# ruc-aimc-lab/GeoFormer

Measured on NVIDIA B200. Metric: pairs_per_sec_640x480, higher is better.
Workload: dtype tf32 / fp16 tensor-core operands with fp32 accumulation (fp32 residual stream, fp16 intermediates), split-fp16 similarity, f16 backbone activations

## Files before the change

geoformer_b200/_lib.py:

```python
from __future__ import annotations

import ctypes
import os
from ctypes import c_char_p, c_float, c_int, c_int64, c_void_p

HERE = os.path.dirname(os.path.abspath(__file__))
LIB_PATH = os.path.join(HERE, "libgeoformer_sm100.so")

P, I, L, F = c_void_p, c_int, c_int64, c_float

SIGNATURES = {
    "gf_abi_version": (I, []),
    "gf_last_error": (c_char_p, []),
    "gf_init": (I, [I]),
    "gf_launch_count": (L, []),
    "gf_linear_tf32": (I, [P, P, P, P, L, I, I, I, I, I, P, P, I, P, P, P, P, P]),
    "gf_linear_ref": (I, [P, P, P, P, L, I, I, I, I, I, P, P, I, P, P, P, P, P]),
    "gf_conv3x3_f16": (I, [P, P, P, P, P, I, I, I, I, I, I, I, P]),
    "gf_conv_f16": (I, [P, P, P, P, P, I, I, I, I, I, I, I, I, I, P]),
    "gf_stem_conv7x7_f16": (I, [P, P, P, P, I, I, I, P]),
    "gf_upsample_add_f16": (I, [P, P, P, I, I, I, I, I, I, P]),
    "gf_conv_ref": (I, [P, P, P, P, P, I, I, I, I, I, I, I, I, P]),
    "gf_upsample_add_ref": (I, [P, P, P, I, I, I, I, I, I, P]),
    "gf_add_posenc": (I, [P, P, P, I, L, I, P]),
    "gf_linattn_partial_floats": (L, [I, I, I, I]),
    "gf_linear_mixed": (I, [P, P, P, P, I, I, L, I, I, I, I, I, P, P, I, P, P, P, P, P]),
    "gf_fine_layer": (I, [P, P, P, P, P, P, P, P, L, P]),
    "gf_linattn_reduce_f16": (I, [P, I, P, I, I, I, I, I, P, P, P, P]),
    "gf_linattn_apply_f16": (I, [P, I, P, P, P, I, I, I, I, I, P]),
    "gf_linattn_window_f16": (I, [P, I, P, I, P, I, P, L, I, I, I, P]),
    "gf_linattn_reduce": (I, [P, I, P, I, I, I, I, I, P, P, P, P]),
    "gf_linattn_apply": (I, [P, I, P, P, P, I, I, I, I, I, P]),
    "gf_linattn_window": (I, [P, I, P, I, P, I, P, L, I, I, I, P]),
    "gf_pack_split_f16": (I, [P, P, L, I, F, I, P]),
    "gf_similarity_f16x3": (I, [P, P, P, I, I, I, I, F, P]),
    "gf_similarity_ref": (I, [P, P, P, I, I, I, I, F, F, P]),
    "gf_dual_softmax_workspace_floats": (L, [I, I, I]),
    "gf_dual_softmax_stats": (I, [P, I, I, I, P, P, P, P, P, P]),
    "gf_dual_softmax_conf": (I, [P, I, I, I, P, P, P, P, P, P, P]),
    "gf_conf_row_col_max": (I, [P, I, I, I, P, P, P]),
    "gf_mnn_select": (I, [P, I, I, I, F, I, I, I, I, I, P, P, P, P, P]),
    "gf_coarse_match_fused_workspace_bytes": (L, [I, I, I]),
    "gf_coarse_match_fused": (I, [P, P, I, I, I, I, F, F, I, I, I, I, I, P, P, P, P]),
    "gf_coarse_match_fused_pass": (I, [P, P, I, I, I, I, F, P, I, P]),
    "gf_compact_coarse": (I, [P, P, I, I, I, I, F, P, P, P, P, P, P, P, P, L, P]),
    "gf_geo_window_table": (I, [P, P, I, I, I, I, I, I, I, I, P, P]),
    "gf_geo_self_attention": (I, [P, I, P, I, P, I, P, I, I, I, I, P, P, I, P]),
    "gf_gather_anchor_kv": (I, [P, I, P, I, I, I, I, I, P, P, I, I, P, P, P]),
    "gf_gather_anchor_kv_f16": (I, [P, I, P, I, P, I, I, I, I, I, P, P, I, I, P, P, P, P]),
    "gf_geo_self_attention_tc": (I, [P, I, P, P, P, I, I, I, I, I, P, P]),
    "gf_gather_anchor_kv_h16": (I, [P, I, P, I, I, I, I, I, P, P, I, I, P, P, P]),
    "gf_masked_softmax_rows": (I, [P, I, I, I, I, P, P]),
    "gf_gemm_tf32_batched": (I, [P, L, L, P, L, L, P, L, L, I, I, I, I, F, P]),
    "gf_geo_cross_attention": (I, [P, I, P, I, P, I, P, I, I, I, I, I, P, I, P]),
    "gf_geo_cross_attention_f16": (I, [P, I, P, I, P, I, P, I, I, I, I, I, P, I, P]),
    "gf_select_rows": (I, [P, P, P, I, L, I, P]),
    "gf_fine_gather": (I, [P, I, I, I, P, P, L, I, I, I, P, P]),
# ... 60 lines not shown
```

geoformer_b200/csrc/conv_tc.cu:

```cuda
#include "common.cuh"
#include "ptx.cuh"

#include <atomic>
#include <cstdlib>
#include <cuda_fp16.h>

namespace gf {
extern std::atomic<int64_t> g_launches;

struct ConvParams {
  const float* bias;
  const __half* residual;
  int batch, h, w, cout_p;
  int kbc;
  int last_k;
  int tail;
  int taps, stride, pad;
  int tiles_x, tiles_y;
  int act;
};

template <int BN, int MT = 1> struct ConvCfg {
  static constexpr int kStageA = MT * 128 * 128;
  static constexpr int kStageB = (BN / 2) * 128;
// ... 253 lines not shown
                                         float ry, float rx) {
  const int64_t idx = (int64_t)blockIdx.x * blockDim.x + threadIdx.x;
  const int64_t total = (int64_t)b * h * w * c8;
  if (idx >= total) return;
  const int ch = (int)(idx % c8);
  int64_t r = idx / c8;
  const int x = (int)(r % w); r /= w;
  const int y = (int)(r % h);
  const int n = (int)(r / h);
  const float fy = ry * y, fx = rx * x;
  const int y0 = (int)fy, x0 = (int)fx;
  const int y1 = min(y0 + 1, hs - 1), x1 = min(x0 + 1, ws - 1);
  const float ly = fy - y0, lx = fx - x0;
  const float w00 = (1.f - ly) * (1.f - lx), w01 = (1.f - ly) * lx, w10 = ly * (1.f - lx), w11 = ly * lx;
  const uint4* s = src + (int64_t)n * hs * ws * c8;
  const uint4 a = __ldg(s + ((int64_t)y0 * ws + x0) * c8 + ch), bq = __ldg(s + ((int64_t)y0 * ws + x1) * c8 + ch);
  const uint4 cq = __ldg(s + ((int64_t)y1 * ws + x0) * c8 + ch), d = __ldg(s + ((int64_t)y1 * ws + x1) * c8 + ch);
  const uint4 l = __ldg(lateral + idx);
  const uint32_t aw[4] = {a.x, a.y, a.z, a.w}, bw[4] = {bq.x, bq.y, bq.z, bq.w}, cw[4] = {cq.x, cq.y, cq.z, cq.w},
                 dw[4] = {d.x, d.y, d.z, d.w}, lw[4] = {l.x, l.y, l.z, l.w};
  uint32_t o[4];
#pragma unroll
  for (int q = 0; q < 4; ++q) {
    const __half2 a2 = *reinterpret_cast<const __half2*>(&aw[q]), b2 = *reinterpret_cast<const __half2*>(&bw[q]);
    const __half2 c2 = *reinterpret_cast<const __half2*>(&cw[q]), d2 = *reinterpret_cast<const __half2*>(&dw[q]);
    const __half2 l2 = *reinterpret_cast<const __half2*>(&lw[q]);
    const float lo = __low2float(l2) + w00 * __low2float(a2) + w01 * __low2float(b2) + w10 * __low2float(c2) + w11 * __low2float(d2);
    const float hi = __high2float(l2) + w00 * __high2float(a2) + w01 * __high2float(b2) + w10 * __high2float(c2) + w11 * __high2float(d2);
    o[q] = pack_f16(lo, hi);
  }
  out[idx] = make_uint4(o[0], o[1], o[2], o[3]);
}

__global__ void __launch_bounds__(256)
stem_conv7x7_kernel(const float* __restrict__ img, const float* __restrict__ wperm, const float* __restrict__ bias,
                    __half* __restrict__ out, int h, int w, int ho, int wo) {
  __shared__ float patch[21][72];
  __shared__ __align__(16) float ws[49 * 128];
  const int b = blockIdx.z;
  const int oy0 = blockIdx.y * 8, ox0 = blockIdx.x * 32;
  const int tid = threadIdx.x;
  for (int e = tid; e < 49 * 128; e += 256) ws[e] = wperm[e];
  const int iy0 = oy0 * 2 - 3, ix0 = ox0 * 2 - 3;
  const float* im = img + (int64_t)b * h * w;
  for (int e = tid; e < 21 * 69; e += 256) {
    const int r = e / 69, c = e - r * 69;
    const int y = iy0 + r, x = ix0 + c;
    patch[r][c] = (y >= 0 && y < h && x >= 0 && x < w) ? im[(int64_t)y * w + x] : 0.f;
  }
  __syncthreads();
  const int cg = tid & 7, pg = tid >> 3;
  const int prow = pg >> 2, pcol = (pg & 3) * 8;
  float acc[8][16];
#pragma unroll
  for (int i = 0; i < 8; ++i)
#pragma unroll
    for (int j = 0; j < 16; ++j) acc[i][j] = 0.f;
#pragma unroll 1
  for (int ky = 0; ky < 7; ++ky) {
    float in[21];
#pragma unroll
    for (int i = 0; i < 21; ++i) in[i] = patch[prow * 2 + ky][pcol * 2 + i];
#pragma unroll
    for (int kx = 0; kx < 7; ++kx) {
      const float4* wp = reinterpret_cast<const float4*>(ws + (ky * 7 + kx) * 128) + cg;
#pragma unroll
      for (int j = 0; j < 4; ++j) {
        const float4 w4 = wp[j * 8];
#pragma unroll
        for (int i = 0; i < 8; ++i) {
          const float x = in[2 * i + kx];
          acc[i][4 * j] = fmaf(x, w4.x, acc[i][4 * j]); acc[i][4 * j + 1] = fmaf(x, w4.y, acc[i][4 * j + 1]);
          acc[i][4 * j + 2] = fmaf(x, w4.z, acc[i][4 * j + 2]); acc[i][4 * j + 3] = fmaf(x, w4.w, acc[i][4 * j + 3]);
        }
      }
    }
  }
  const int oy = oy0 + prow;
  if (oy < ho) {
#pragma unroll
    for (int j = 0; j < 4; ++j) {
      const float4 b4 = __ldg(reinterpret_cast<const float4*>(bias + j * 32 + cg * 4));
#pragma unroll
      for (int i = 0; i < 8; ++i) {
        const int ox = ox0 + pcol + i;
        if (ox < wo) {
          uint2 o;
          o.x = pack_f16(fmaxf(acc[i][4 * j] + b4.x, 0.f), fmaxf(acc[i][4 * j + 1] + b4.y, 0.f));
          o.y = pack_f16(fmaxf(acc[i][4 * j + 2] + b4.z, 0.f), fmaxf(acc[i][4 * j + 3] + b4.w, 0.f));
          *reinterpret_cast<uint2*>(out + (((int64_t)b * ho + oy) * wo + ox) * 128 + j * 32 + cg * 4) = o;
        }
      }
    }
  }
}

typedef CUresult (*EncodeTiledFn)(CUtensorMap*, CUtensorMapDataType, cuuint32_t, void*, const cuuint64_t*,
                                  const cuuint64_t*, const cuuint32_t*, const cuuint32_t*, CUtensorMapInterleave,
                                  CUtensorMapSwizzle, CUtensorMapL2promotion, CUtensorMapFloatOOBfill);
EncodeTiledFn encode_fn();

static int make_nhwc_tmap(CUtensorMap* m, const void* base, int c, int w, int h, int b, int box_w, int box_h, int stride = 1,
                          int box_c = 64) {
  EncodeTiledFn enc = encode_fn();
  if (!enc) return gf_set_error(GF_ERR_DRIVER, "gf_init() was not called");
  cuuint64_t dims[4] = {(cuuint64_t)c, (cuuint64_t)w, (cuuint64_t)h, (cuuint64_t)b};
  cuuint64_t strides[3] = {(cuuint64_t)c * 2, (cuuint64_t)c * 2 * w, (cuuint64_t)c * 2 * w * h};
  cuuint32_t box[4] = {(cuuint32_t)box_c, (cuuint32_t)(box_w * stride), (cuuint32_t)(box_h * stride), 1};
  cuuint32_t estr[4] = {1, (cuuint32_t)stride, (cuuint32_t)stride, 1};
  CUresult r = enc(m, CU_TENSOR_MAP_DATA_TYPE_FLOAT16, 4, const_cast<void*>(base), dims, strides, box, estr,
                   CU_TENSOR_MAP_INTERLEAVE_NONE, box_c == 64 ? CU_TENSOR_MAP_SWIZZLE_128B : CU_TENSOR_MAP_SWIZZLE_32B,
                   CU_TENSOR_MAP_L2_PROMOTION_L2_256B, CU_TENSOR_MAP_FLOAT_OOB_FILL_NONE);
  if (r != CUDA_SUCCESS) return gf_set_error(GF_ERR_DRIVER, "cuTensorMapEncodeTiled(nhwc) failed");
  return GF_OK;
}

static int make_wtail_tmap(CUtensorMap* m, const void* base, int64_t k, int64_t rows, int box_rows) {
  EncodeTiledFn enc = encode_fn();
  if (!enc) return gf_set_error(GF_ERR_DRIVER, "gf_init() was not called");
  cuuint64_t dims[3] = {(cuuint64_t)k, (cuuint64_t)rows, 1};
  cuuint64_t strides[2] = {(cuuint64_t)k * 2, (cuuint64_t)k * 2 * (cuuint64_t)rows};
  cuuint32_t box[3] = {16, (cuuint32_t)box_rows, 1};
  cuuint32_t estr[3] = {1, 1, 1};
// ... 55 lines not shown
    if ((rc = make_wtail_tmap(&twt, wt, taps * (int64_t)cin_k, cout_p, BN / 2))) return rc;
  }
  p.tiles_x = gf_cdiv(wo, 16); p.tiles_y = gf_cdiv(ho, 8); p.act = act;
  if (BN == 128 && ho >= 32 && getenv("GF_CONV_MT1") == nullptr) {
    p.tiles_y = gf_cdiv(ho, 16);
    return launch_conv<128, 2>(tx, tw, ty, txt, twt, p, (cudaStream_t)stream);
  }
  if (BN == 128) return launch_conv<128>(tx, tw, ty, txt, twt, p, (cudaStream_t)stream);
  if (BN == 208) return launch_conv<208>(tx, tw, ty, txt, twt, p, (cudaStream_t)stream);
  return launch_conv<256>(tx, tw, ty, txt, twt, p, (cudaStream_t)stream);
}

extern "C" int gf_conv3x3_f16(const void* x, const void* wt, const float* bias, const void* residual, void* y,
                               int batch, int h, int w, int cin_p, int cout_p, int cin_k, int act, gf_stream_t stream) {
  return gf_conv_f16(x, wt, bias, residual, y, batch, h, w, cin_p, cout_p, cin_k, 3, 1, act, stream);
}

extern "C" int gf_upsample_add_f16(const void* lateral, const void* src, void* out, int batch, int h, int w, int hs,
                                    int ws, int c, gf_stream_t stream) {
  if (batch <= 0 || h <= 1 || w <= 1 || hs <= 0 || ws <= 0 || (c % 8)) return gf_set_error(GF_ERR_ARG, "gf_upsample_add_f16: bad shape");
  const int64_t total = (int64_t)batch * h * w * (c / 8);
  const float ry = (float)(hs - 1) / (float)(h - 1), rx = (float)(ws - 1) / (float)(w - 1);
  upsample_add_f16_kernel<<<gf_cdiv(total, 256), 256, 0, (cudaStream_t)stream>>>(
      (const uint4*)lateral, (const uint4*)src, (uint4*)out, batch, h, w, hs, ws, c / 8, ry, rx);
  g_launches++;
  GF_CHECK_LAUNCH();
  return GF_OK;
}

extern "C" int gf_stem_conv7x7_f16(const float* img, const float* wperm, const float* bias, void* out, int batch, int h,
                                    int w, gf_stream_t stream) {
  if (batch <= 0 || h <= 0 || w <= 0) return gf_set_error(GF_ERR_ARG, "gf_stem_conv7x7_f16: bad shape");
  const int ho = (h + 6 - 7) / 2 + 1, wo = (w + 6 - 7) / 2 + 1;
  stem_conv7x7_kernel<<<dim3(gf_cdiv(wo, 32), gf_cdiv(ho, 8), batch), 256, 0, (cudaStream_t)stream>>>(
      img, wperm, bias, (__half*)out, h, w, ho, wo);
  g_launches++;
  GF_CHECK_LAUNCH();
  return GF_OK;
}
```

geoformer_b200/csrc/linattn.cu:

```cuda
#include "common.cuh"

#include <cuda_fp16.h>

#include <atomic>

namespace gf {
extern std::atomic<int64_t> g_launches;

template <typename T> __device__ __forceinline__ float4 ld4(const T* p);
template <> __device__ __forceinline__ float4 ld4<float>(const float* p) { return *reinterpret_cast<const float4*>(p); }
template <> __device__ __forceinline__ float4 ld4<__half>(const __half* p) {
  const uint2 u = *reinterpret_cast<const uint2*>(p);
  const float2 a = __half22float2(*reinterpret_cast<const __half2*>(&u.x));
  const float2 b = __half22float2(*reinterpret_cast<const __half2*>(&u.y));
  return make_float4(a.x, a.y, b.x, b.y);
}
__device__ __forceinline__ void st1(float* p, float v) { *p = v; }
__device__ __forceinline__ void st1(__half* p, float v) { *p = __float2half_rn(v); }

constexpr int kChunk = 256;
constexpr int kChunkMma = 128;

template <int D, typename T>
__global__ void linattn_partial_kernel(const T* __restrict__ K, int ldk, const T* __restrict__ V, int ldv,
// ... 407 lines not shown
  __syncthreads();
  float ksr[D];
#pragma unroll
  for (int d = 0; d < D; ++d) ksr[d] = ksum[h * D + d];
  __half* os = reinterpret_cast<__half*>(vs);
#pragma unroll 5
  for (int r = 0; r < TOK; ++r) {
    const float4* qr = reinterpret_cast<const float4*>(qs + r * c + h * D);
    float num = 0.f, den = 0.f;
#pragma unroll
    for (int q = 0; q < D / 4; ++q) {
      const float4 q4 = qr[q];
      num = fmaf(q4.x, kvcol[4 * q], num); den = fmaf(q4.x, ksr[4 * q], den);
      num = fmaf(q4.y, kvcol[4 * q + 1], num); den = fmaf(q4.y, ksr[4 * q + 1], den);
      num = fmaf(q4.z, kvcol[4 * q + 2], num); den = fmaf(q4.z, ksr[4 * q + 2], den);
      num = fmaf(q4.w, kvcol[4 * q + 3], num); den = fmaf(q4.w, ksr[4 * q + 3], den);
    }
    os[r * c + t] = __float2half_rn(num * (1.f / (den + 1e-6f)) * ftok);
  }
  __syncthreads();
  uint4* dst = reinterpret_cast<uint4*>(out + w * (TOK * c));
  const uint4* src = reinterpret_cast<const uint4*>(os);
  for (int i = t; i < TOK * c / 8; i += 128) dst[i] = src[i];
}

__global__ void add_posenc_kernel(const float4* __restrict__ x, const float4* __restrict__ pe, float4* __restrict__ out,
                                  int64_t per_sample4, int64_t total4) {
  const int64_t i = (int64_t)blockIdx.x * blockDim.x + threadIdx.x;
  if (i >= total4) return;
  const float4 a = x[i], b = pe[i % per_sample4];
  out[i] = make_float4(a.x + b.x, a.y + b.y, a.z + b.z, a.w + b.w);
}

__global__ void select_rows_kernel(float4* __restrict__ dst, const float4* __restrict__ src, const int* __restrict__ flag,
                                   int64_t per_sample4, int64_t total4) {
  const int64_t i = (int64_t)blockIdx.x * blockDim.x + threadIdx.x;
  if (i >= total4) return;
  if (flag[i / per_sample4] == 0) dst[i] = src[i];
}

__global__ void gather_rows_kernel(const float* __restrict__ feat, int64_t l, int c, const int64_t* __restrict__ b_ids,
                                   const int64_t* __restrict__ tok, int64_t m, float* __restrict__ out) {
  const int64_t i = (int64_t)blockIdx.x * blockDim.x + threadIdx.x;
  const int c4 = c >> 2;
  if (i >= m * c4) return;
  const int64_t r = i / c4;
  const int q = (int)(i - r * c4);
  const float4* src = reinterpret_cast<const float4*>(feat + (b_ids[r] * l + tok[r]) * c);
  reinterpret_cast<float4*>(out)[i] = src[q];
}

}

using namespace gf;
#define STREAM ((cudaStream_t)stream)

extern "C" int64_t gf_linattn_partial_floats(int n, int s, int heads, int dim) {
  return (int64_t)n * heads * gf_cdiv(s, kChunkMma) * (dim * dim + dim);
}

template <typename T>
static int linattn_reduce_impl(const T* K, int ldk, const T* V, int ldv, int n, int s, int heads, int dim,
                               float* partial, float* KV, float* Ksum, gf_stream_t stream) {
  if (n <= 0 || s <= 0 || heads <= 0 || heads > 32 || dim != 32 || (ldk % 4) || (ldv % 4))
    return gf_set_error(GF_ERR_ARG, "gf_linattn_reduce: dim must be 32, heads <= 32, 16-byte aligned rows");
  const int nchunks = gf_cdiv(s, kChunk);
// ... 65 lines not shown
  linattn_window16_kernel<16, 25><<<(unsigned)n_windows, 128, smem, STREAM>>>((const __half*)Q, ldq, (const __half*)K, ldk,
                                                                            (const __half*)V, ldv, (__half*)out);
  g_launches++;
  GF_CHECK_LAUNCH();
  return GF_OK;
}

extern "C" int gf_linattn_window(const float* Q, int ldq, const float* K, int ldk, const float* V, int ldv, float* out,
                                 int64_t n_windows, int tokens, int heads, int dim, gf_stream_t stream) {
  const int c = heads * dim;
  if (n_windows < 0 || tokens <= 0 || tokens > 64 || dim != 16 || c > 1024 || (c % 32))
    return gf_set_error(GF_ERR_ARG, "gf_linattn_window: dim must be 16");
  if (n_windows == 0) return GF_OK;
  const size_t smem = (size_t)(3 * tokens * c + c) * sizeof(float);
  GF_SMEM_OPTIN((linattn_window_kernel<16, 0>), 96 * 1024);
  GF_SMEM_OPTIN((linattn_window_kernel<16, 25>), 96 * 1024);
  if (smem > 96 * 1024) return gf_set_error(GF_ERR_ARG, "gf_linattn_window: shared memory");
  if (tokens == 25) linattn_window_kernel<16, 25><<<(unsigned)n_windows, c, smem, STREAM>>>(Q, ldq, K, ldk, V, ldv, out, tokens, heads);
  else              linattn_window_kernel<16, 0><<<(unsigned)n_windows, c, smem, STREAM>>>(Q, ldq, K, ldk, V, ldv, out, tokens, heads);
  g_launches++;
  GF_CHECK_LAUNCH();
  return GF_OK;
}

extern "C" int gf_add_posenc(const float* x, const float* pe, float* out, int n, int64_t l, int c, gf_stream_t stream) {
  if (n <= 0 || l <= 0 || c <= 0 || (c % 4)) return gf_set_error(GF_ERR_ARG, "gf_add_posenc: bad shape");
  const int64_t per = l * c / 4, total = per * n;
  add_posenc_kernel<<<gf_cdiv(total, 256), 256, 0, STREAM>>>((const float4*)x, (const float4*)pe, (float4*)out, per, total);
  g_launches++;
  GF_CHECK_LAUNCH();
  return GF_OK;
}

extern "C" int gf_select_rows(float* dst, const float* src, const int* flag, int n, int64_t l, int c, gf_stream_t stream) {
  if (n <= 0 || l <= 0 || c <= 0 || (c % 4)) return gf_set_error(GF_ERR_ARG, "gf_select_rows: bad shape");
  const int64_t per = l * c / 4, total = per * n;
  select_rows_kernel<<<gf_cdiv(total, 256), 256, 0, STREAM>>>((float4*)dst, (const float4*)src, flag, per, total);
  g_launches++;
  GF_CHECK_LAUNCH();
  return GF_OK;
}

extern "C" int gf_gather_rows(const float* feat, int64_t l, int c, const int64_t* b_ids, const int64_t* tok_ids,
                              int64_t m, float* out, gf_stream_t stream) {
  if (m < 0 || c <= 0 || (c % 4)) return gf_set_error(GF_ERR_ARG, "gf_gather_rows: bad shape");
  if (m == 0) return GF_OK;
  gather_rows_kernel<<<gf_cdiv(m * (c / 4), 256), 256, 0, STREAM>>>(feat, l, c, b_ids, tok_ids, m, out);
  g_launches++;
  GF_CHECK_LAUNCH();
  return GF_OK;
}
```

geoformer_b200/engine.py:

```python
from __future__ import annotations

import math
import os
import threading
from concurrent.futures import ThreadPoolExecutor
from typing import Dict, List, Optional, Tuple

import numpy as np
import torch

from . import ops
from .ops import EPI_ELU1, EPI_LN, EPI_RELU, EPI_TANH

_POOL: Optional[ThreadPoolExecutor] = None
FUSED_MATCHING = os.environ.get("GF_FUSED_MATCHING", "1") != "0"
FUSED_FINE_LAYER = os.environ.get("GF_FUSED_FINE", "1") != "0"


def _pool() -> ThreadPoolExecutor:
    global _POOL
    if _POOL is None:
        ranks = max(1, int(os.environ.get("LOCAL_WORLD_SIZE", "1")))
        nthr = int(os.environ.get("GF_RANSAC_THREADS", "0")) or max(2, min(16, (os.cpu_count() or 2) // ranks))
        _POOL = ThreadPoolExecutor(max_workers=nthr)
# ... 116 lines not shown
        elif backbone_dtype == torch.float32:
            r = {}
            for name, bn in names:
                w, b = folded(name, bn)
                co, ci, kh, kw = w.shape
                r[key(name)] = (w.permute(2, 3, 1, 0).reshape(kh * kw, ci, co).contiguous().to(device),
                                None if b is None else b.to(device))
            self.bb_ref = r
        else:
            raise ValueError(f"backbone dtype must be float16 (product) or float32 (accurate), got {backbone_dtype}")
        self._pe: Dict[Tuple[int, int, int], torch.Tensor] = {}
        self._pe_lock = threading.Lock()

    def pos_table(self, c: int, h: int, w: int) -> torch.Tensor:
        key = (c, h, w)
        t = self._pe.get(key)
        if t is not None:
            return t
        with self._pe_lock:
            if key in self._pe:
                return self._pe[key]
            ypos = torch.ones(h, w).cumsum(0).float().unsqueeze(0)
            xpos = torch.ones(h, w).cumsum(1).float().unsqueeze(0)
            div = torch.exp(torch.arange(0, c // 2, 2).float() * (-math.log(10000.0) / c // 2))[:, None, None]
            pe = torch.zeros(c, h, w)
            pe[0::4] = torch.sin(xpos * div); pe[1::4] = torch.cos(xpos * div)
            pe[2::4] = torch.sin(ypos * div); pe[3::4] = torch.cos(ypos * div)
            t = pe.permute(1, 2, 0).reshape(h * w, c).contiguous().to(self.device)
            torch.cuda.current_stream(self.device).synchronize()
            self._pe[key] = t
        return t


def backbone_forward(pw: PackedWeights, img: torch.Tensor) -> Tuple[torch.Tensor, torch.Tensor]:
    return backbone_forward_tc(pw, img) if pw.bb_tc is not None else backbone_forward_ref(pw, img)


def backbone_forward_ref(pw: PackedWeights, img: torch.Tensor) -> Tuple[torch.Tensor, torch.Tensor]:
    r = pw.bb_ref

    def conv(name, t, act, residual=None, stride=1):
        wt, b = r[name]
        return ops.conv_ref(t, wt, b, residual, act, stride)

    def block(p, a):
        if (p + ".down") in r:
            y = conv(p + ".conv1", a, 1, stride=2)
            a = conv(p + ".down", a, 0, stride=2)
        else:
            y = conv(p + ".conv1", a, 1)
        return conv(p + ".conv2", y, 1, residual=a)

    b, _, h, w = img.shape
    x0 = conv("conv1", img.contiguous().view(b, h, w, 1), 1, stride=2)
    x1 = block("layer1.1", block("layer1.0", x0))
    x2 = block("layer2.1", block("layer2.0", x1))
    x3 = block("layer3.1", block("layer3.0", x2))
    x3o = conv("layer3_outconv", x3, 0)
    x2o = ops.upsample_add_ref(conv("layer2_outconv", x2, 0), x3o)
    x2o = conv("layer2_outconv2.3", conv("layer2_outconv2.0", x2o, 2), 0)
    x1o = ops.upsample_add_ref(conv("layer1_outconv", x1, 0), x2o)
    x1o = conv("layer1_outconv2.3", conv("layer1_outconv2.0", x1o, 2), 0)
    return x3o, x1o


def backbone_forward_tc(pw: PackedWeights, img: torch.Tensor) -> Tuple[torch.Tensor, torch.Tensor]:
    tc = pw.bb_tc

    def conv(name, t, act, residual=None, stride=1):
        wt, b = tc[name]
        return ops.conv(t, wt, b, residual, act, stride)

    def block(p, a):
        if (p + ".down") in tc:
            y = conv(p + ".conv1", a, 1, stride=2)
            a = conv(p + ".down", a, 0, stride=2)
        else:
            y = conv(p + ".conv1", a, 1)
        return conv(p + ".conv2", y, 1, residual=a)

    x0 = ops.stem_conv(img.contiguous(), *tc["stem"])
    x1 = block("layer1.1", block("layer1.0", x0))
    x2 = block("layer2.1", block("layer2.0", x1))
    x3 = block("layer3.1", block("layer3.0", x2))
    x3o = conv("layer3_outconv", x3, 0)
    x2o = ops.upsample_add(conv("layer2_outconv", x2, 0), x3o)
    x2o = conv("layer2_outconv2.3", conv("layer2_outconv2.0", x2o, 2), 0)
    x1o = ops.upsample_add(conv("layer1_outconv", x1, 0), x2o)
    x1o = conv("layer1_outconv2.3", conv("layer1_outconv2.0", x1o, 2), 0)
    return x3o.float().contiguous(), x1o


def _post_attention(lw: dict, x2d: torch.Tensor, msg: torch.Tensor, act: int, out: Optional[torch.Tensor] = None) -> torch.Tensor:
    h16 = ops.act16()
    m1 = ops.linear(msg, lw["wm16"] if msg.dtype == torch.float16 else lw["wm"], epi=EPI_LN, gamma=lw["n1w"], beta=lw["n1b"])
    h = ops.linear(x2d, lw["w1"], a2=m1, epi=act, out_f16=h16)
    return ops.linear(h, lw["w2_16"] if h16 else lw["w2"], epi=EPI_LN, gamma=lw["n2w"], beta=lw["n2b"], residual=x2d, out=out)


def loftr_layer(lw: dict, x: torch.Tensor, src: torch.Tensor, heads: int, out: Optional[torch.Tensor] = None,
                q_mask: Optional[torch.Tensor] = None, kv_mask: Optional[torch.Tensor] = None) -> torch.Tensor:
    n, l, c = x.shape
    s = src.shape[1]
    d = c // heads
    x2d = x.reshape(n * l, c)
    a16 = ops.act16()
    if x is src:
        qkv = ops.linear(x2d, lw["wqkv"], epi=EPI_ELU1, act_cols=2 * c, out_f16=a16)
        if q_mask is not None and q_mask is kv_mask:
            ops.mask_rows_(qkv, q_mask)
        else:
            if q_mask is not None:
                ops.mask_rows_(qkv, q_mask, 0, c)
            if kv_mask is not None:
                ops.mask_rows_(qkv, kv_mask, c, 2 * c)
        q, k, v, ldq, ldk = qkv, qkv[:, c:], qkv[:, 2 * c:], 3 * c, 3 * c
    else:
        q = ops.linear(x2d, lw["wq"], epi=EPI_ELU1, act_cols=c, out_f16=a16)
        kv = ops.linear(src.reshape(n * s, c), lw["wkv"], epi=EPI_ELU1, act_cols=c, out_f16=a16)
        if q_mask is not None:
            ops.mask_rows_(q, q_mask)
        if kv_mask is not None:
            ops.mask_rows_(kv, kv_mask)
        k, v, ldq, ldk = kv, kv[:, c:], c, 2 * c
    msg = ops.linattn(q, ldq, k, ldk, v, ldk, n, l, s, heads, d)
    return _post_attention(lw, x2d, msg, EPI_RELU, None if out is None else out.view(n * l, c)).view(n, l, c)


def coarse_transformer(pw: PackedWeights, x0: torch.Tensor, x1: torch.Tensor, names, heads: int,
                       mask0: Optional[torch.Tensor] = None, mask1: Optional[torch.Tensor] = None):
    n = x0.shape[0]
    same = x0.shape == x1.shape
    assert (mask0 is None) == (mask1 is None), "padding masks come in pairs (full_model.py:82-83)"
    mm = None
    if same:
        X = torch.cat([x0, x1], 0)
        x0, x1 = X[:n], X[n:]
        if mask0 is not None:
            mm = torch.cat([mask0, mask1], 0)
    for lw, name in zip(pw.coarse, names):
        if name == "self":
            if same:
                X = loftr_layer(lw, X, X, heads, q_mask=mm, kv_mask=mm)
                x0, x1 = X[:n], X[n:]
            else:
                x0 = loftr_layer(lw, x0, x0, heads, q_mask=mask0, kv_mask=mask0)
                x1 = loftr_layer(lw, x1, x1, heads, q_mask=mask1, kv_mask=mask1)
        elif same:
            Xn = torch.empty_like(X)
            y0 = loftr_layer(lw, x0, x1, heads, out=Xn[:n], q_mask=mask0, kv_mask=mask1)
            loftr_layer(lw, x1, y0, heads, out=Xn[n:], q_mask=mask1, kv_mask=mask0)
            X = Xn
            x0, x1 = X[:n], X[n:]
        else:
            y0 = loftr_layer(lw, x0, x1, heads, q_mask=mask0, kv_mask=mask1)
            x0, x1 = y0, loftr_layer(lw, x1, y0, heads, q_mask=mask1, kv_mask=mask0)
    return x0, x1


def fine_layer(lw: dict, x: torch.Tensor, src: torch.Tensor, heads: int) -> torch.Tensor:
    m, t, c = x.shape
    d = c // heads
    if FUSED_FINE_LAYER and ops.act16() and (t, c, heads) == (25, 128, 8) and "wpack" in lw:
        return ops.fine_layer_fused(x.contiguous(), src.contiguous(), lw["wpack"], lw["n1w"], lw["n1b"], lw["n2w"], lw["n2b"])
    x2d = x.reshape(m * t, c)
    a16 = ops.act16() and t == 25 and heads == 8 and d == 16
    if x is src:
        qkv = ops.linear(x2d, lw["wqkv"], epi=EPI_ELU1, act_cols=2 * c, out_f16=a16)
        q, k, v, ldq, ldk = qkv, qkv[:, c:], qkv[:, 2 * c:], 3 * c, 3 * c
# ... 188 lines not shown
```

geoformer_b200/model/full_model.py:

```python
from __future__ import annotations

import os
import threading
from typing import Dict, Optional

import torch
import torch.nn as nn

from geoformer_b200 import engine, ops
from .geo_config import default_cfg


def _conv(cin, cout, k):
    return nn.Conv2d(cin, cout, kernel_size=k, bias=False)


class _Block(nn.Module):
    def __init__(self, cin, cout, stride):
        super().__init__()
        self.conv1, self.conv2 = _conv(cin, cout, 3), _conv(cout, cout, 3)
        self.bn1, self.bn2 = nn.BatchNorm2d(cout), nn.BatchNorm2d(cout)
        self.downsample = None if stride == 1 else nn.Sequential(_conv(cin, cout, 1), nn.BatchNorm2d(cout))


# ... 114 lines not shown
                                         (pw.fine, cfg["fine"]["layer_names"], "fine"), (pw.geo, gcfg["layer_names"], "geo")):
                    assert len(got) == len(names), f"{what}: {len(got)} layers in the state dict, {len(names)} in the config"
                torch.cuda.current_stream(device).synchronize()
                self._packed = pw
            return self._packed

    @torch.no_grad()
    def forward(self, data: Dict[str, torch.Tensor]):
        img0, img1 = data["image0"], data["image1"]
        if (data.get("mask0") is None) != (data.get("mask1") is None):
            raise ValueError("geoformer_b200.GeoFormer: padding masks come in pairs (mask0 AND mask1)")
        for k in ("scale0", "scale1", "dataset_name"):
            if data.get(k) is not None:
                raise NotImplementedError(f"geoformer_b200.GeoFormer: data[{k!r}] is not supported (training-only key)")
        if not img0.is_cuda:
            raise RuntimeError("geoformer_b200.GeoFormer runs on CUDA (sm_100a) only; there is no CPU fallback")
        with torch.cuda.device(img0.device):
            if self.precision:
                with ops.precision_scope(**self.precision):
                    return self._forward(data, img0, img1)
            return self._forward(data, img0, img1)

    def _forward(self, data, img0, img1):
        pw = self._weights(img0.device)
        cfg, gcfg = self.config, self.geo_cfg
        n = img0.shape[0]
        hw0_i, hw1_i = tuple(img0.shape[2:]), tuple(img1.shape[2:])
        data.update({"bs": torch.tensor(n), "hw0_i": torch.tensor(hw0_i), "hw1_i": torch.tensor(hw1_i)})
        stages = {} if self.capture else None

        R = ops.PROFILE.region
        with R("stage:backbone"):
            if hw0_i == hw1_i:
                c, f = engine.backbone_forward(pw, torch.cat([img0, img1], 0))
                c0, c1, f0, f1 = c[:n], c[n:], f[:n], f[n:]
            else:
                (c0, f0), (c1, f1) = engine.backbone_forward(pw, img0), engine.backbone_forward(pw, img1)
        hw0_c, hw1_c, hw0_f, hw1_f = tuple(c0.shape[1:3]), tuple(c1.shape[1:3]), tuple(f0.shape[1:3]), tuple(f1.shape[1:3])
        data.update({"hw0_c": torch.tensor(hw0_c), "hw1_c": torch.tensor(hw1_c),
                     "hw0_f": torch.tensor(hw0_f), "hw1_f": torch.tensor(hw1_f)})
        dc = c0.shape[-1]

        mk0 = mk1 = None
        if data.get("mask0") is not None:
            mk0 = ops.token_mask(data["mask0"], n, hw0_c[0] * hw0_c[1])
            mk1 = ops.token_mask(data["mask1"], n, hw1_c[0] * hw1_c[1])
        with R("stage:coarse_transformer"):
            x0 = ops.add_posenc(c0.reshape(n, -1, dc), pw.pos_table(dc, *hw0_c))
            x1 = ops.add_posenc(c1.reshape(n, -1, dc), pw.pos_table(dc, *hw1_c))
            t0, t1 = engine.coarse_transformer(pw, x0, x1, cfg["coarse"]["layer_names"], cfg["coarse"]["nhead"], mk0, mk1)

        thr = cfg["match_coarse"]["thr"]
        temp = cfg["match_coarse"]["dsmax_temperature"]
        with R("stage:coarse_matching_1"):
            m1, counts1, conf1 = engine.coarse_matching(t0.contiguous(), t1.contiguous(), thr, temp, 0, hw0_i, hw0_c,
                                                        hw1_c, self.materialize, mk0, mk1)
        ginfo = {} if self.capture else None
        with R("stage:geo_module(+host RANSAC)"):
            g0, g1 = engine.geo_module(pw, x0, x1, m1, counts1, hw0_i, hw1_i, hw0_c, hw1_c, gcfg["layer_names"],
                                       gcfg["nhead"], gcfg["window_size"], info=ginfo, ransac=self.ransac,
                                       ransac_hyps=self.ransac_hyps)
        with R("stage:coarse_matching_2"):
            m2, counts2, conf2 = engine.coarse_matching(g0, g1, thr, temp, 0, hw0_i, hw0_c, hw1_c, self.materialize,
                                                        mk0, mk1)
        data.update(m2)
        if self.materialize:
            data.update({"dect_conf_matrix": conf1, "conf_matrix": conf2})

        w = cfg["fine_window_size"]
        data.update({"W": torch.tensor(w)})
        if m2["b_ids"].shape[0] == 0:
            data.update({"mkpts0_f": m2["mkpts0_c"], "mkpts1_f": m2["mkpts1_c"],
                         "fine_matrix": torch.empty(0, w * w, w * w, device=img0.device)})
            fstages = {}
        else:
            with R("stage:fine"):
                out, fmat, fstages = engine.fine_stage(pw, f0, f1, g0, g1, m2, hw0_i, hw0_c, hw1_c, hw0_f, w,
                                                       cfg["fine"]["nhead"], cfg["fine"]["layer_names"],
                                                       gcfg["fine_temperature"], gcfg["fine_thr"], self.materialize)
            data.update(out)
            if self.materialize:
                data["fine_matrix"] = fmat
        if stages is not None:
            stages.update(cnn_c0=c0, cnn_c1=c1, fine0=f0, fine1=f1, pe0=x0, pe1=x1, coarse0=t0, coarse1=t1,
                          first=m1, counts_first=counts1, geo0=g0, geo1=g1, geo_info=ginfo, counts=counts2, **fstages)
            data["_stages"] = stages
        return data
```

geoformer_b200/ops.py:

```python
from __future__ import annotations

import os
import threading
from typing import Optional, Tuple

import torch

from . import _lib

EPI_RELU, EPI_TANH, EPI_ELU1, EPI_LN = 1, 2, 4, 8

_LINEAR_IMPL = "tf32"
_SIM_IMPL = "f16x3"
_ATTN_IMPL = "tf32"
_ACT16 = os.environ.get("GF_ACT16", "1") != "0"


def act16() -> bool:
    return _ACT16 and _LINEAR_IMPL == "tf32"


def set_precision(linear: Optional[str] = None, similarity: Optional[str] = None,
                  attention: Optional[str] = None, activations: Optional[str] = None) -> None:
    global _LINEAR_IMPL, _SIM_IMPL, _ATTN_IMPL, _ACT16
# ... 200 lines not shown
          c, _stream())
    return out


def conv_ref(x: torch.Tensor, wt: torch.Tensor, bias: Optional[torch.Tensor], residual: Optional[torch.Tensor] = None,
             act: int = 0, stride: int = 1) -> torch.Tensor:
    _chk(x); _chk(wt)
    assert x.is_contiguous() and wt.is_contiguous()
    b, h, w, cin = x.shape
    taps, cin_w, cout = wt.shape
    k = {1: 1, 9: 3, 49: 7}[taps]
    assert cin_w == cin
    pad = k // 2
    y = torch.empty((b, (h + 2 * pad - k) // stride + 1, (w + 2 * pad - k) // stride + 1, cout), device=x.device)
    if residual is not None:
        assert residual.shape == y.shape and residual.is_contiguous() and residual.dtype == torch.float32
    _call("gf_conv_ref", x.data_ptr(), wt.data_ptr(), _ptr(bias), _ptr(residual), y.data_ptr(), b, h, w, cin, cout, k,
          stride, act, _stream(), tag=f"[{cin}->{cout}@{h}x{w}k{k}s{stride}]")
    return y


def upsample_add_ref(lateral: torch.Tensor, src: torch.Tensor) -> torch.Tensor:
    _chk(lateral); _chk(src)
    assert lateral.is_contiguous() and src.is_contiguous()
    b, h, w, c = lateral.shape
    out = torch.empty_like(lateral)
    _call("gf_upsample_add_ref", lateral.data_ptr(), src.data_ptr(), out.data_ptr(), b, h, w, src.shape[1], src.shape[2],
          c, _stream())
    return out


def add_posenc(x: torch.Tensor, pe: torch.Tensor) -> torch.Tensor:
    n, l, c = x.shape
    assert x.is_contiguous() and pe.is_contiguous() and pe.shape == (l, c)
    out = torch.empty_like(x)
    _call("gf_add_posenc", x.data_ptr(), pe.data_ptr(), out.data_ptr(), n, l, c, _stream())
    return out


def token_mask(mask: torch.Tensor, n: int, tokens: int) -> torch.Tensor:
    if not mask.is_cuda:
        raise _lib.GeoFormerLibError("geoformer_b200 ops need CUDA tensors (no CPU fallback)")
    if mask.shape[0] != n or mask[0].numel() != tokens:
        raise ValueError(f"padding mask of shape {tuple(mask.shape)} does not cover {n} x {tokens} coarse tokens")
    m = mask.reshape(n, tokens)
    return (m if m.dtype == torch.bool else m != 0).contiguous().view(torch.uint8)


def mask_rows_(buf: torch.Tensor, mask: torch.Tensor, col0: int = 0, cols: Optional[int] = None) -> torch.Tensor:
    assert buf.dim() == 2 and buf.is_contiguous() and buf.dtype in (torch.float32, torch.float16)
    assert mask.dtype == torch.uint8 and mask.is_contiguous() and mask.numel() == buf.shape[0] and mask.device == buf.device
    rows, ld = buf.shape
    cols = ld - col0 if cols is None else cols
    _call("gf_mask_rows", buf.data_ptr(), buf.element_size(), rows, ld, col0, cols, mask.data_ptr(), _stream())
    return buf


def mask_fill_sim_(sim: torch.Tensor, mask0: torch.Tensor, mask1: torch.Tensor, fill: float = -1e9) -> torch.Tensor:
    _chk(sim)
    n, l, s = sim.shape
    assert sim.is_contiguous() and mask0.dtype == mask1.dtype == torch.uint8
    assert tuple(mask0.shape) == (n, l) and tuple(mask1.shape) == (n, s) and mask0.is_contiguous() and mask1.is_contiguous()
    _call("gf_mask_fill_sim", sim.data_ptr(), n, l, s, mask0.data_ptr(), mask1.data_ptr(), float(fill), _stream())
    return sim


def linattn(q: torch.Tensor, ldq: int, k: torch.Tensor, ldk: int, v: torch.Tensor, ldv: int, n: int, l: int, s: int,
            heads: int, dim: int) -> torch.Tensor:
    dev = q.device
# ... 267 lines not shown
```

include/geoformer_b200.h:

```cpp
#ifndef GEOFORMER_B200_H_
#define GEOFORMER_B200_H_

#include <stdint.h>

#ifdef __cplusplus
extern "C" {
#endif

#define GF_ABI_VERSION 1

#define GF_OK 0
#define GF_ERR_ARG (-1)
#define GF_ERR_LAUNCH (-2)
#define GF_ERR_DRIVER (-3)
#define GF_ERR_DEVICE (-4)

#define GF_EPI_RELU 1
#define GF_EPI_TANH 2
#define GF_EPI_ELU1 4
#define GF_EPI_LN 8

typedef void* gf_stream_t;

int gf_abi_version(void);
const char* gf_last_error(void);
int gf_init(int device);
int64_t gf_launch_count(void);

int gf_linear_tf32(const float* A, const float* A2, const float* W, float* Y, int64_t M, int N, int K1, int K2,
                   int epi, int act_cols, const float* bias, const float* rowbias, int rowbias_group,
                   const float* gamma, const float* beta, const float* residual, const int* m_dev,
                   gf_stream_t stream);
int gf_linear_mixed(const void* A, const void* A2, const void* W, void* Y, int in_f16, int out_f16, int64_t M, int N,
                    int K1, int K2, int epi, int act_cols, const float* bias, const float* rowbias, int rowbias_group,
                    const float* gamma, const float* beta, const float* residual, const int* m_dev, gf_stream_t stream);
int gf_linear_ref(const float* A, const float* A2, const float* W, float* Y, int64_t M, int N, int K1, int K2,
                  int epi, int act_cols, const float* bias, const float* rowbias, int rowbias_group,
                  const float* gamma, const float* beta, const float* residual, const int* m_dev,
                  gf_stream_t stream);

int gf_conv3x3_f16(const void* x, const void* wt, const float* bias, const void* residual, void* y, int batch, int h,
                    int w, int cin_p, int cout_p, int cin_k, int act, gf_stream_t stream);
int gf_conv_f16(const void* x, const void* wt, const float* bias, const void* residual, void* y, int batch, int h, int w,
                 int cin_p, int cout_p, int cin_k, int ksize, int stride, int act, gf_stream_t stream);

int gf_stem_conv7x7_f16(const float* img, const float* wperm, const float* bias, void* out, int batch, int h, int w,
                         gf_stream_t stream);
int gf_upsample_add_f16(const void* lateral, const void* src, void* out, int batch, int h, int w, int hs, int ws,
                         int c, gf_stream_t stream);
int gf_conv_ref(const float* x, const float* wt, const float* bias, const float* residual, float* y, int batch, int h,
                int w, int cin, int cout, int ksize, int stride, int act, gf_stream_t stream);
int gf_upsample_add_ref(const float* lateral, const float* src, float* out, int batch, int h, int w, int hs, int ws,
                        int c, gf_stream_t stream);

int gf_add_posenc(const float* x, const float* pe, float* out, int n, int64_t l, int c, gf_stream_t stream);

int64_t gf_linattn_partial_floats(int n, int s, int heads, int dim);
int gf_linattn_reduce(const float* K, int ldk, const float* V, int ldv, int n, int s, int heads, int dim,
                      float* partial, float* KV, float* Ksum, gf_stream_t stream);
int gf_linattn_apply(const float* Q, int ldq, const float* KV, const float* Ksum, float* out, int n, int l, int s,
                     int heads, int dim, gf_stream_t stream);
int gf_linattn_window(const float* Q, int ldq, const float* K, int ldk, const float* V, int ldv, float* out,
                      int64_t n_windows, int tokens, int heads, int dim, gf_stream_t stream);
int gf_linattn_reduce_f16(const void* K, int ldk, const void* V, int ldv, int n, int s, int heads, int dim,
                          float* partial, float* KV, float* Ksum, gf_stream_t stream);
int gf_linattn_apply_f16(const void* Q, int ldq, const float* KV, const float* Ksum, void* out, int n, int l, int s,
                         int heads, int dim, gf_stream_t stream);
int gf_linattn_window_f16(const void* Q, int ldq, const void* K, int ldk, const void* V, int ldv, void* out,
                          int64_t n_windows, int tokens, int heads, int dim, gf_stream_t stream);

int gf_pack_split_f16(const float* x, void* out_f16, int64_t rows, int c, float scale, int role, gf_stream_t stream);
int gf_similarity_f16x3(const void* a3, const void* b3, float* sim, int n, int l, int s, int c3, float out_scale,
                        gf_stream_t stream);
int gf_similarity_ref(const float* f0, const float* f1, float* sim, int n, int l, int s, int c, float in_scale,
                      float out_scale, gf_stream_t stream);
int64_t gf_dual_softmax_workspace_floats(int n, int l, int s);
int gf_dual_softmax_stats(const float* sim, int n, int l, int s, float* row_max, float* row_sum, float* col_max,
                          float* col_sum, float* workspace, gf_stream_t stream);
int gf_dual_softmax_conf(float* sim_conf, int n, int l, int s, const float* row_max, const float* row_sum,
                         const float* col_max, const float* col_sum, float* conf_row_max, float* conf_col_max,
                         gf_stream_t stream);
int gf_conf_row_col_max(const float* conf, int n, int l, int s, float* conf_row_max, float* conf_col_max,
                        gf_stream_t stream);
int gf_mnn_select(const float* conf, int n, int l, int s, float thr, int border, int h0c, int w0c, int h1c, int w1c,
                  const float* conf_row_max, const float* conf_col_max, int* match_j, float* match_conf,
                  gf_stream_t stream);
int64_t gf_coarse_match_fused_workspace_bytes(int n, int l, int s);
int gf_coarse_match_fused(const void* a3, const void* b3, int n, int l, int s, int c3, float out_scale, float thr,
// ... 72 lines not shown
```

Measured before the change: 469.9.

## Persist stem conv with async double-buffered patches; fuse f16 upcast into posenc

The 7x7 stem conv becomes a persistent kernel with one block per SM and 512 threads. Each block loops over tiles and prefetches the next input patch with cp.async into a second shared buffer, so the weight table is loaded once per block instead of once per tile, at the cost of higher register and shared memory pressure. The backbone now returns the coarse map in fp16, and a new add_posenc_f16 kernel converts it and adds the positional encoding in one pass over both images together. This drops the separate .float() copy, two posenc launches and the torch.cat before the coarse transformer.

```diff
diff --git a/geoformer_b200/_lib.py b/geoformer_b200/_lib.py
--- a/geoformer_b200/_lib.py
+++ b/geoformer_b200/_lib.py
@@ -23,6 +23,7 @@
     "gf_conv_ref": (I, [P, P, P, P, P, I, I, I, I, I, I, I, I, P]),
     "gf_upsample_add_ref": (I, [P, P, P, I, I, I, I, I, I, P]),
     "gf_add_posenc": (I, [P, P, P, I, L, I, P]),
+    "gf_add_posenc_f16": (I, [P, P, P, I, L, I, P]),
     "gf_linattn_partial_floats": (L, [I, I, I, I]),
     "gf_linear_mixed": (I, [P, P, P, P, I, I, L, I, I, I, I, I, P, P, I, P, P, P, P, P]),
     "gf_fine_layer": (I, [P, P, P, P, P, P, P, P, L, P]),
diff --git a/geoformer_b200/csrc/conv_tc.cu b/geoformer_b200/csrc/conv_tc.cu
--- a/geoformer_b200/csrc/conv_tc.cu
+++ b/geoformer_b200/csrc/conv_tc.cu
@@ -309,63 +309,84 @@
   out[idx] = make_uint4(o[0], o[1], o[2], o[3]);
 }
 
-__global__ void __launch_bounds__(256)
+constexpr int kStemThreads = 512, kStemPatchRows = 21, kStemPatchCols = 69, kStemPatchLd = 72;
+
+__device__ __forceinline__ void stem_fetch_patch(float* patch, const float* __restrict__ img, int t, int tiles_x,
+                                                 int tiles_per_img, int h, int w) {
+  const int b = t / tiles_per_img, r = t - b * tiles_per_img;
+  const int iy0 = (r / tiles_x) * 16 - 3, ix0 = (r % tiles_x) * 64 - 3;
+  const float* im = img + (int64_t)b * h * w;
+  for (int e = threadIdx.x; e < kStemPatchRows * kStemPatchCols; e += kStemThreads) {
+    const int pr = e / kStemPatchCols, pc = e - pr * kStemPatchCols;
+    const int y = iy0 + pr, x = ix0 + pc;
+    const bool in = y >= 0 && y < h && x >= 0 && x < w;
+    const float* src = in ? im + (int64_t)y * w + x : img;
+    asm volatile("cp.async.ca.shared.global [%0], [%1], 4, %2;"
+                 ::"r"(ptx::smem_addr(patch + pr * kStemPatchLd + pc)), "l"(src), "r"(in ? 4 : 0) : "memory");
+  }
+  asm volatile("cp.async.commit_group;" ::: "memory");
+}
+
+__global__ void __launch_bounds__(kStemThreads, 1)
 stem_conv7x7_kernel(const float* __restrict__ img, const float* __restrict__ wperm, const float* __restrict__ bias,
-                    __half* __restrict__ out, int h, int w, int ho, int wo) {
-  __shared__ float patch[21][72];
+                    __half* __restrict__ out, int h, int w, int ho, int wo, int tiles_x, int tiles_per_img,
+                    int total_tiles) {
+  __shared__ __align__(16) float patches[2][kStemPatchRows * kStemPatchLd];
   __shared__ __align__(16) float ws[49 * 128];
-  const int b = blockIdx.z;
-  const int oy0 = blockIdx.y * 8, ox0 = blockIdx.x * 32;
   const int tid = threadIdx.x;
-  for (int e = tid; e < 49 * 128; e += 256) ws[e] = wperm[e];
-  const int iy0 = oy0 * 2 - 3, ix0 = ox0 * 2 - 3;
-  const float* im = img + (int64_t)b * h * w;
-  for (int e = tid; e < 21 * 69; e += 256) {
-    const int r = e / 69, c = e - r * 69;
-    const int y = iy0 + r, x = ix0 + c;
-    patch[r][c] = (y >= 0 && y < h && x >= 0 && x < w) ? im[(int64_t)y * w + x] : 0.f;
-  }
-  __syncthreads();
-  const int cg = tid & 7, pg = tid >> 3;
+  if ((int)blockIdx.x < total_tiles) stem_fetch_patch(patches[0], img, blockIdx.x, tiles_x, tiles_per_img, h, w);
+  for (int e = tid; e < 49 * 128; e += kStemThreads) ws[e] = __ldg(wperm + e);
+  const int cg = tid & 15, pg = tid >> 4;
   const int prow = pg >> 2, pcol = (pg & 3) * 8;
-  float acc[8][16];
-#pragma unroll
-  for (int i = 0; i < 8; ++i)
-#pragma unroll
-    for (int j = 0; j < 16; ++j) acc[i][j] = 0.f;
+  int buf = 0;
 #pragma unroll 1
-  for (int ky = 0; ky < 7; ++ky) {
-    float in[21];
-#pragma unroll
-    for (int i = 0; i < 21; ++i) in[i] = patch[prow * 2 + ky][pcol * 2 + i];
-#pragma unroll
-    for (int kx = 0; kx < 7; ++kx) {
-      const float4* wp = reinterpret_cast<const float4*>(ws + (ky * 7 + kx) * 128) + cg;
-#pragma unroll
-      for (int j = 0; j < 4; ++j) {
-        const float4 w4 = wp[j * 8];
-#pragma unroll
-        for (int i = 0; i < 8; ++i) {
-          const float x = in[2 * i + kx];
-          acc[i][4 * j] = fmaf(x, w4.x, acc[i][4 * j]); acc[i][4 * j + 1] = fmaf(x, w4.y, acc[i][4 * j + 1]);
-          acc[i][4 * j + 2] = fmaf(x, w4.z, acc[i][4 * j + 2]); acc[i][4 * j + 3] = fmaf(x, w4.w, acc[i][4 * j + 3]);
+  for (int t = blockIdx.x; t < total_tiles; t += gridDim.x, buf ^= 1) {
+    asm volatile("cp.async.wait_all;" ::: "memory");
+    __syncthreads();
+    if (t + (int)gridDim.x < total_tiles)
+      stem_fetch_patch(patches[buf ^ 1], img, t + gridDim.x, tiles_x, tiles_per_img, h, w);
+    const float* patch = patches[buf];
+    const int b = t / tiles_per_img, r = t - b * tiles_per_img;
+    const int oy0 = (r / tiles_x) * 8, ox0 = (r % tiles_x) * 32;
+    float acc[8][8];
+#pragma unroll
+    for (int i = 0; i < 8; ++i)
+#pragma unroll
+      for (int j = 0; j < 8; ++j) acc[i][j] = 0.f;
+#pragma unroll 1
+    for (int ky = 0; ky < 7; ++ky) {
+      float in[21];
+#pragma unroll
+      for (int i = 0; i < 21; ++i) in[i] = patch[(prow * 2 + ky) * kStemPatchLd + pcol * 2 + i];
+#pragma unroll
+      for (int kx = 0; kx < 7; ++kx) {
+        const float4* wp = reinterpret_cast<const float4*>(ws + (ky * 7 + kx) * 128) + cg;
+#pragma unroll
+        for (int j = 0; j < 2; ++j) {
+          const float4 w4 = wp[j * 16];
+#pragma unroll
+          for (int i = 0; i < 8; ++i) {
+            const float x = in[2 * i + kx];
+            acc[i][4 * j] = fmaf(x, w4.x, acc[i][4 * j]); acc[i][4 * j + 1] = fmaf(x, w4.y, acc[i][4 * j + 1]);
+            acc[i][4 * j + 2] = fmaf(x, w4.z, acc[i][4 * j + 2]); acc[i][4 * j + 3] = fmaf(x, w4.w, acc[i][4 * j + 3]);
+          }
         }
       }
     }
-  }
-  const int oy = oy0 + prow;
-  if (oy < ho) {
-#pragma unroll
-    for (int j = 0; j < 4; ++j) {
-      const float4 b4 = __ldg(reinterpret_cast<const float4*>(bias + j * 32 + cg * 4));
-#pragma unroll
-      for (int i = 0; i < 8; ++i) {
-        const int ox = ox0 + pcol + i;
-        if (ox < wo) {
-          uint2 o;
-          o.x = pack_f16(fmaxf(acc[i][4 * j] + b4.x, 0.f), fmaxf(acc[i][4 * j + 1] + b4.y, 0.f));
-          o.y = pack_f16(fmaxf(acc[i][4 * j + 2] + b4.z, 0.f), fmaxf(acc[i][4 * j + 3] + b4.w, 0.f));
-          *reinterpret_cast<uint2*>(out + (((int64_t)b * ho + oy) * wo + ox) * 128 + j * 32 + cg * 4) = o;
+    const int oy = oy0 + prow;
+    if (oy < ho) {
+#pragma unroll
+      for (int j = 0; j < 2; ++j) {
+        const float4 b4 = __ldg(reinterpret_cast<const float4*>(bias + j * 64 + cg * 4));
+#pragma unroll
+        for (int i = 0; i < 8; ++i) {
+          const int ox = ox0 + pcol + i;
+          if (ox < wo) {
+            uint2 o;
+            o.x = pack_f16(fmaxf(acc[i][4 * j] + b4.x, 0.f), fmaxf(acc[i][4 * j + 1] + b4.y, 0.f));
+            o.y = pack_f16(fmaxf(acc[i][4 * j + 2] + b4.z, 0.f), fmaxf(acc[i][4 * j + 3] + b4.w, 0.f));
+            *reinterpret_cast<uint2*>(out + (((int64_t)b * ho + oy) * wo + ox) * 128 + j * 64 + cg * 4) = o;
+          }
         }
       }
     }
@@ -487,8 +508,10 @@
                                     int w, gf_stream_t stream) {
   if (batch <= 0 || h <= 0 || w <= 0) return gf_set_error(GF_ERR_ARG, "gf_stem_conv7x7_f16: bad shape");
   const int ho = (h + 6 - 7) / 2 + 1, wo = (w + 6 - 7) / 2 + 1;
-  stem_conv7x7_kernel<<<dim3(gf_cdiv(wo, 32), gf_cdiv(ho, 8), batch), 256, 0, (cudaStream_t)stream>>>(
-      img, wperm, bias, (__half*)out, h, w, ho, wo);
+  const int tiles_x = gf_cdiv(wo, 32), tiles_per_img = tiles_x * gf_cdiv(ho, 8);
+  const int total = batch * tiles_per_img, grid = total < num_sms() ? total : num_sms();
+  stem_conv7x7_kernel<<<grid, kStemThreads, 0, (cudaStream_t)stream>>>(img, wperm, bias, (__half*)out, h, w, ho, wo,
+                                                                       tiles_x, tiles_per_img, total);
   g_launches++;
   GF_CHECK_LAUNCH();
   return GF_OK;
diff --git a/geoformer_b200/csrc/linattn.cu b/geoformer_b200/csrc/linattn.cu
--- a/geoformer_b200/csrc/linattn.cu
+++ b/geoformer_b200/csrc/linattn.cu
@@ -463,6 +463,19 @@
   out[i] = make_float4(a.x + b.x, a.y + b.y, a.z + b.z, a.w + b.w);
 }
 
+__global__ void add_posenc_f16_kernel(const uint4* __restrict__ x, const float4* __restrict__ pe, float4* __restrict__ out,
+                                      int64_t per_sample8, int64_t total8) {
+  const int64_t i = (int64_t)blockIdx.x * blockDim.x + threadIdx.x;
+  if (i >= total8) return;
+  const uint4 a = x[i];
+  const int64_t j = i % per_sample8;
+  const float4 p0 = pe[2 * j], p1 = pe[2 * j + 1];
+  const float2 a0 = __half22float2(*reinterpret_cast<const __half2*>(&a.x)), a1 = __half22float2(*reinterpret_cast<const __half2*>(&a.y));
+  const float2 a2 = __half22float2(*reinterpret_cast<const __half2*>(&a.z)), a3 = __half22float2(*reinterpret_cast<const __half2*>(&a.w));
+  out[2 * i] = make_float4(a0.x + p0.x, a0.y + p0.y, a1.x + p0.z, a1.y + p0.w);
+  out[2 * i + 1] = make_float4(a2.x + p1.x, a2.y + p1.y, a3.x + p1.z, a3.y + p1.w);
+}
+
 __global__ void select_rows_kernel(float4* __restrict__ dst, const float4* __restrict__ src, const int* __restrict__ flag,
                                    int64_t per_sample4, int64_t total4) {
   const int64_t i = (int64_t)blockIdx.x * blockDim.x + threadIdx.x;
@@ -594,6 +607,15 @@
   return GF_OK;
 }
 
+extern "C" int gf_add_posenc_f16(const void* x, const float* pe, float* out, int n, int64_t l, int c, gf_stream_t stream) {
+  if (n <= 0 || l <= 0 || c <= 0 || (c % 8)) return gf_set_error(GF_ERR_ARG, "gf_add_posenc_f16: bad shape");
+  const int64_t per = l * c / 8, total = per * n;
+  add_posenc_f16_kernel<<<gf_cdiv(total, 256), 256, 0, STREAM>>>((const uint4*)x, (const float4*)pe, (float4*)out, per, total);
+  g_launches++;
+  GF_CHECK_LAUNCH();
+  return GF_OK;
+}
+
 extern "C" int gf_select_rows(float* dst, const float* src, const int* flag, int n, int64_t l, int c, gf_stream_t stream) {
   if (n <= 0 || l <= 0 || c <= 0 || (c % 4)) return gf_set_error(GF_ERR_ARG, "gf_select_rows: bad shape");
   const int64_t per = l * c / 4, total = per * n;
diff --git a/geoformer_b200/engine.py b/geoformer_b200/engine.py
--- a/geoformer_b200/engine.py
+++ b/geoformer_b200/engine.py
@@ -172,8 +172,8 @@
         return t
 
 
-def backbone_forward(pw: PackedWeights, img: torch.Tensor) -> Tuple[torch.Tensor, torch.Tensor]:
-    return backbone_forward_tc(pw, img) if pw.bb_tc is not None else backbone_forward_ref(pw, img)
+def backbone_forward(pw: PackedWeights, img: torch.Tensor, coarse_f16: bool = False) -> Tuple[torch.Tensor, torch.Tensor]:
+    return backbone_forward_tc(pw, img, coarse_f16) if pw.bb_tc is not None else backbone_forward_ref(pw, img)
 
 
 def backbone_forward_ref(pw: PackedWeights, img: torch.Tensor) -> Tuple[torch.Tensor, torch.Tensor]:
@@ -204,7 +204,7 @@
     return x3o, x1o
 
 
-def backbone_forward_tc(pw: PackedWeights, img: torch.Tensor) -> Tuple[torch.Tensor, torch.Tensor]:
+def backbone_forward_tc(pw: PackedWeights, img: torch.Tensor, coarse_f16: bool = False) -> Tuple[torch.Tensor, torch.Tensor]:
     tc = pw.bb_tc
 
     def conv(name, t, act, residual=None, stride=1):
@@ -228,7 +228,7 @@
     x2o = conv("layer2_outconv2.3", conv("layer2_outconv2.0", x2o, 2), 0)
     x1o = ops.upsample_add(conv("layer1_outconv", x1, 0), x2o)
     x1o = conv("layer1_outconv2.3", conv("layer1_outconv2.0", x1o, 2), 0)
-    return x3o.float().contiguous(), x1o
+    return (x3o if coarse_f16 else x3o.float().contiguous()), x1o
 
 
 def _post_attention(lw: dict, x2d: torch.Tensor, msg: torch.Tensor, act: int, out: Optional[torch.Tensor] = None) -> torch.Tensor:
@@ -267,6 +267,14 @@
     return _post_attention(lw, x2d, msg, EPI_RELU, None if out is None else out.view(n * l, c)).view(n, l, c)
 
 
+def _halves_of(x0: torch.Tensor, x1: torch.Tensor) -> Optional[torch.Tensor]:
+    X = x0._base
+    if X is None or x1._base is not X or not X.is_contiguous() or X.shape != (2 * x0.shape[0], *x0.shape[1:]):
+        return None
+    half = x0.numel() * x0.element_size()
+    return X if x0.data_ptr() == X.data_ptr() and x1.data_ptr() == X.data_ptr() + half else None
+
+
 def coarse_transformer(pw: PackedWeights, x0: torch.Tensor, x1: torch.Tensor, names, heads: int,
                        mask0: Optional[torch.Tensor] = None, mask1: Optional[torch.Tensor] = None):
     n = x0.shape[0]
@@ -274,7 +282,9 @@
     assert (mask0 is None) == (mask1 is None), "padding masks come in pairs (full_model.py:82-83)"
     mm = None
     if same:
-        X = torch.cat([x0, x1], 0)
+        X = _halves_of(x0, x1)
+        if X is None:
+            X = torch.cat([x0, x1], 0)
         x0, x1 = X[:n], X[n:]
         if mask0 is not None:
             mm = torch.cat([mask0, mask1], 0)
diff --git a/geoformer_b200/model/full_model.py b/geoformer_b200/model/full_model.py
--- a/geoformer_b200/model/full_model.py
+++ b/geoformer_b200/model/full_model.py
@@ -170,7 +170,7 @@
         R = ops.PROFILE.region
         with R("stage:backbone"):
             if hw0_i == hw1_i:
-                c, f = engine.backbone_forward(pw, torch.cat([img0, img1], 0))
+                c, f = engine.backbone_forward(pw, torch.cat([img0, img1], 0), coarse_f16=True)
                 c0, c1, f0, f1 = c[:n], c[n:], f[:n], f[n:]
             else:
                 (c0, f0), (c1, f1) = engine.backbone_forward(pw, img0), engine.backbone_forward(pw, img1)
@@ -184,8 +184,12 @@
             mk0 = ops.token_mask(data["mask0"], n, hw0_c[0] * hw0_c[1])
             mk1 = ops.token_mask(data["mask1"], n, hw1_c[0] * hw1_c[1])
         with R("stage:coarse_transformer"):
-            x0 = ops.add_posenc(c0.reshape(n, -1, dc), pw.pos_table(dc, *hw0_c))
-            x1 = ops.add_posenc(c1.reshape(n, -1, dc), pw.pos_table(dc, *hw1_c))
+            if hw0_i == hw1_i and mk0 is None and c.dtype == torch.float16:
+                X = ops.add_posenc(c.reshape(2 * n, -1, dc), pw.pos_table(dc, *hw0_c))
+                x0, x1 = X[:n], X[n:]
+            else:
+                x0 = ops.add_posenc(c0.float().reshape(n, -1, dc), pw.pos_table(dc, *hw0_c))
+                x1 = ops.add_posenc(c1.float().reshape(n, -1, dc), pw.pos_table(dc, *hw1_c))
             t0, t1 = engine.coarse_transformer(pw, x0, x1, cfg["coarse"]["layer_names"], cfg["coarse"]["nhead"], mk0, mk1)
 
         thr = cfg["match_coarse"]["thr"]
@@ -220,7 +224,7 @@
             if self.materialize:
                 data["fine_matrix"] = fmat
         if stages is not None:
-            stages.update(cnn_c0=c0, cnn_c1=c1, fine0=f0, fine1=f1, pe0=x0, pe1=x1, coarse0=t0, coarse1=t1,
+            stages.update(cnn_c0=c0.float(), cnn_c1=c1.float(), fine0=f0, fine1=f1, pe0=x0, pe1=x1, coarse0=t0, coarse1=t1,
                           first=m1, counts_first=counts1, geo0=g0, geo1=g1, geo_info=ginfo, counts=counts2, **fstages)
             data["_stages"] = stages
         return data
diff --git a/geoformer_b200/ops.py b/geoformer_b200/ops.py
--- a/geoformer_b200/ops.py
+++ b/geoformer_b200/ops.py
@@ -256,9 +256,11 @@
 
 def add_posenc(x: torch.Tensor, pe: torch.Tensor) -> torch.Tensor:
     n, l, c = x.shape
+    assert x.dtype in (torch.float32, torch.float16)
     assert x.is_contiguous() and pe.is_contiguous() and pe.shape == (l, c)
-    out = torch.empty_like(x)
-    _call("gf_add_posenc", x.data_ptr(), pe.data_ptr(), out.data_ptr(), n, l, c, _stream())
+    out = torch.empty((n, l, c), device=x.device, dtype=torch.float32)
+    _call("gf_add_posenc_f16" if x.dtype == torch.float16 else "gf_add_posenc", x.data_ptr(), pe.data_ptr(),
+          out.data_ptr(), n, l, c, _stream())
     return out
 
 
diff --git a/include/geoformer_b200.h b/include/geoformer_b200.h
--- a/include/geoformer_b200.h
+++ b/include/geoformer_b200.h
@@ -54,6 +54,7 @@
                         int c, gf_stream_t stream);
 
 int gf_add_posenc(const float* x, const float* pe, float* out, int n, int64_t l, int c, gf_stream_t stream);
+int gf_add_posenc_f16(const void* x, const float* pe, float* out, int n, int64_t l, int c, gf_stream_t stream);
 
 int64_t gf_linattn_partial_floats(int n, int s, int heads, int dim);
 int gf_linattn_reduce(const float* K, int ldk, const float* V, int ldv, int n, int s, int heads, int dim,
```

After: 475.1, median of 6. 1.1% higher.
